# Frikallo/parakeet.cpp

Hardware: AMD Instinct MI355X
Metric: RTFx (audio-sec/wall-sec), mel+encoder+TDT decode, tdt-ctc-110m 10s@b64 (higher is better)
Workload: dtype f32; 1 GPU; tdt-ctc-110m, batch=64x10s clips per GPU, TDT greedy decode (the loops of 4 consecutive steps driven as one lock-step batch), fp32 (BASELINE configs[1]); parallelism=dp1 (utterance shards, no data-path collective), decode_group=4, decode_loop=phases, decode_overlap=1

## Files before the change

include/parakeet_amd.h:

```cpp
#ifndef PARAKEET_AMD_H
#define PARAKEET_AMD_H

#include <stddef.h>
#include <stdint.h>

#ifdef __cplusplus
extern "C" {
#endif

typedef int pk_status;
enum {
    PK_OK = 0,
    PK_ERR_INVALID = -1,
    PK_ERR_IO = -2,
    PK_ERR_WEIGHTS = -3,
    PK_ERR_NO_DEVICE = -4,
    PK_ERR_HIP = -5,
    PK_ERR_DECODE_CAP = -6,
    PK_ERR_UNSUPPORTED = -7
};

typedef struct pk_config {
    int32_t mel_bins;
    int32_t subsampling_channels;
// ... 210 lines not shown
typedef struct pk_sortformer pk_sortformer;
void pk_sortformer_config_preset(pk_sortformer_config *out);
pk_status pk_sortformer_load(const char *safetensors_path, const pk_sortformer_config *cfg, int device, pk_sortformer **out);
void pk_sortformer_free(pk_sortformer *s);
pk_status pk_sortformer_forward(pk_sortformer *s, const float *feats, int B, int Tm, float *probs, int *T_out);
pk_status pk_sortformer_forward_pcm(pk_sortformer *s, const float *pcm, int n_clips, int64_t n_samples, float *probs, int *T_out);
pk_status pk_sortformer_diarize_chunk(pk_sortformer *s, const float *feats, int n_frames, float *probs, int cap_frames, int *T_out);
pk_status pk_sortformer_stream_reset(pk_sortformer *s);
int pk_sortformer_segments(const float *probs, int T, int S, float threshold, int32_t *speaker, float *start, float *end, int cap);

int pk_vocab_size(const pk_model *m);
int pk_detokenize(const pk_model *m, const int32_t *ids, int n, char *out, int cap);
int pk_tokenize(const pk_model *m, const char *text, int32_t *ids, int cap);
pk_status pk_set_boost_tokens(pk_model *m, const int32_t *ids, const int32_t *offsets, int n_phrases, float boost_score);
pk_status pk_set_boost_phrases(pk_model *m, const char *const *phrases, int n_phrases, float boost_score);
int pk_boost_trie_size(const pk_model *m);
int pk_group_timestamps(const pk_model *m, const int32_t *ids, const int32_t *start, const int32_t *end, const float *conf,
                        int n, int sentences, char *words, int cap, float *wstart, float *wend, float *wconf, int wcap);

pk_status pk_diag_math(int fn, const float *in, float *out, int64_t n);
pk_status pk_diag_math_exhaustive(int fn, uint64_t *checked, uint64_t *mismatches, uint64_t *first_bad);
pk_status pk_diag_gemm(int M, int N, int K, const float *A, const float *W, const float *bias, int epi,
                       const float *resid, float alpha, float *out);
pk_status pk_diag_gemm_bf16(int M, int N, int K, const float *A, const float *W, const float *bias, int epi,
                            const float *resid, float alpha, float *out);
pk_status pk_diag_gemm_bf16_a16(int M, int N, int K, const float *A, const float *W, const float *bias, int epi,
                                const float *resid, float alpha, float *out);
pk_status pk_diag_smallm_bf16_tiles(int on);
pk_status pk_diag_ln_gemm_bf16(int M, int N, int K, const float *A, const float *gamma, const float *beta, float eps, const float *W,
                               const float *bias, int epi, const float *resid, float alpha, float *out);
pk_status pk_diag_ln2_gemm_bf16(int M, int N, int K, const float *A, const float *pre_gamma, const float *pre_beta, const float *gamma, const float *beta,
                                float eps, const float *W, const float *bias, float *out, float *pre_out);
pk_status pk_diag_glu_dwconv_bf16(int n_streams, int c, int d, const float *A, const float *gamma, const float *beta, float eps, const float *W,
                                  const float *bias, const float *cache_in, int has_cache, const float *dw_w, const float *dw_bias,
                                  const float *bn_mean, const float *bn_rstd, const float *bn_g, const float *bn_b, int fused, float *out,
                                  float *cache_out);
pk_status pk_diag_ffn_bf16_smallm(int M, int d, int f, const float *x, const float *gamma, const float *beta, float eps, const float *W1, const float *b1,
                                  const float *W2, const float *b2, int act_tiles, float *out);
pk_status pk_diag_layernorm(const float *x, int64_t rows, int d, const float *gamma, const float *beta, float eps, float *y);
pk_status pk_diag_ln_gemm(int M, int N, int K, const float *A, const float *pre_gamma, const float *pre_beta, const float *gamma, const float *beta, float eps,
                          const float *W, const float *bias, int epi, int fold, float *out, float *y1);
pk_status pk_diag_sum64(const float *x, int rows, int n, float *out);
#define PK_DIAG_ATTENTION_GUARD_ROWS 128
pk_status pk_diag_relpos_attention(int kernel, int B, const int32_t *lens, int T, int d, int n_heads, const float *qkv, const float *pos, int pos_T,
                                   const float *bias_u, const float *bias_v, float *ctx, int *variant);
pk_status pk_diag_relpos_local_attention(int B, const int32_t *lens, int T, int d, int n_heads, const float *qkv, const float *pos, int left, int right,
// ... 7 lines not shown
```

parakeet.cpp_amd/capi.py:

```python
import ctypes as C
import os

import numpy as np

from .config import ModelConfig

_HERE = os.path.dirname(os.path.abspath(__file__))
LIB_PATH = os.environ.get("PK_LIB") or os.path.join(_HERE, "libparakeet_amd.so")
_LIB = None

f32p, i32p, i64p = C.POINTER(C.c_float), C.POINTER(C.c_int32), C.POINTER(C.c_int64)


class PkError(RuntimeError):
    def __init__(self, code, msg):
        super().__init__(f"pk_status {code}: {msg}")
        self.code = code


class PkConfig(C.Structure):
    _fields_ = [("mel_bins", C.c_int32), ("subsampling_channels", C.c_int32), ("hidden_size", C.c_int32),
                ("num_layers", C.c_int32), ("num_heads", C.c_int32), ("ffn_intermediate", C.c_int32),
                ("conv_kernel_size", C.c_int32), ("vocab_size", C.c_int32), ("pred_hidden", C.c_int32),
                ("num_lstm_layers", C.c_int32), ("joint_hidden", C.c_int32), ("num_durations", C.c_int32),
# ... 62 lines not shown

def lib():
    global _LIB
    if _LIB is not None:
        return _LIB
    if not os.path.exists(LIB_PATH):
        raise ImportError(f"{LIB_PATH} is missing: run `python -c 'import __graft_entry__ as g; g.build()'` "
                          "(hipcc --offload-arch=gfx950). There is no CPU fallback.")
    L = C.CDLL(LIB_PATH)
    L.pk_version.restype = C.c_char_p
    L.pk_last_error.restype = C.c_size_t
    L.pk_last_error.argtypes = [C.c_char_p, C.c_size_t]
    L.pk_config_preset.argtypes = [C.c_char_p, C.POINTER(PkConfig)]
    L.pk_model_load.argtypes = [C.c_char_p, C.c_char_p, C.POINTER(PkConfig), C.POINTER(C.c_void_p)]
    L.pk_model_to_gpu.argtypes = [C.c_void_p, C.c_int]
    L.pk_model_free.argtypes = [C.c_void_p]
    L.pk_model_config.argtypes = [C.c_void_p, C.POINTER(PkConfig)]
    L.pk_mel.argtypes = [C.c_void_p, f32p, C.c_int, C.c_int64, f32p, f32p]
    L.pk_mel_num_frames.argtypes = [C.c_int64]
    L.pk_encoder_num_frames.argtypes = [C.c_int]
    L.pk_diag_math.argtypes = [C.c_int, f32p, f32p, C.c_int64]
    L.pk_diag_math_exhaustive.argtypes = [C.c_int, C.POINTER(C.c_uint64), C.POINTER(C.c_uint64), C.POINTER(C.c_uint64)]
    L.pk_diag_gemm.argtypes = [C.c_int, C.c_int, C.c_int, f32p, f32p, f32p, C.c_int, f32p, C.c_float, f32p]
    L.pk_diag_gemm_bf16.argtypes = L.pk_diag_gemm.argtypes
    L.pk_diag_gemm_bf16_a16.argtypes = L.pk_diag_gemm.argtypes
    L.pk_diag_layernorm.argtypes = [f32p, C.c_int64, C.c_int, f32p, f32p, C.c_float, f32p]
    L.pk_diag_ln_gemm.argtypes = [C.c_int, C.c_int, C.c_int, f32p, f32p, f32p, f32p, f32p, C.c_float, f32p, f32p, C.c_int, C.c_int, f32p, f32p]
    L.pk_diag_sum64.argtypes = [f32p, C.c_int, C.c_int, f32p]
    L.pk_diag_relpos_attention.argtypes = [C.c_int, C.c_int, i32p, C.c_int, C.c_int, C.c_int, f32p, f32p, C.c_int, f32p, f32p, f32p,
                                           C.POINTER(C.c_int)]
    for name, at in _LATE_SIGNATURES.items():
        if hasattr(L, name):
            getattr(L, name).argtypes = at
    _LIB = L
    return L


_LATE_SIGNATURES = {
    "pk_encode": [C.c_void_p, f32p, C.c_int, C.c_int, C.c_int, C.c_int, f32p],
    "pk_conformer_blocks": [C.c_void_p, f32p, C.c_int, C.c_int, C.c_int, C.c_int, f32p],
    "pk_subsample": [C.c_void_p, f32p, C.c_int, C.c_int, f32p],
    "pk_ctc_decode": [C.c_void_p, f32p, C.c_int, C.c_int, i32p, i32p, i32p, i32p, f32p, f32p],
    "pk_tdt_decode": [C.c_void_p, f32p, C.c_int, C.c_int, C.c_int, i32p, i32p, i32p, i32p, f32p, i32p],
    "pk_model_set_decode_loop": [C.c_void_p, C.c_int],
    "pk_plan_batches": [i64p, C.c_int, i32p, i32p, C.POINTER(C.c_int)],
    "pk_ragged_extents": [i64p, C.c_int, i32p, i32p, i64p],
# ... 156 lines not shown
def read_audio(path, target_rate=16000):
    L = lib()
    L.pk_read_audio.argtypes = [C.c_char_p, C.c_int, C.POINTER(f32p), C.POINTER(C.c_int64), C.POINTER(C.c_int)]
    L.pk_free.argtypes = [C.c_void_p]
    out, n, sr = f32p(), C.c_int64(0), C.c_int(0)
    check(L.pk_read_audio(path.encode(), target_rate, C.byref(out), C.byref(n), C.byref(sr)))
    r = np.ctypeslib.as_array(out, shape=(max(n.value, 1),))[: n.value].copy()
    L.pk_free(out)
    return r, sr.value


def diag_gemm(A, W, bias=None, epi="none", resid=None, alpha=1.0, bf16=False, a16=False):
    A, W = _c(A), _c(W)
    M, K = A.shape
    N = W.shape[0] // 2 if epi == "glu" else W.shape[0]
    b = _c(bias) if bias is not None else None
    r = _c(resid) if resid is not None else None
    out = np.empty((M, N), np.float32)
    fn = (lib().pk_diag_gemm_bf16_a16 if a16 else lib().pk_diag_gemm_bf16) if bf16 else lib().pk_diag_gemm
    check(fn(M, N, K, _f(A), _f(W), _f(b) if b is not None else None, EPI[epi], _f(r) if r is not None else None, alpha, _f(out)))
    return out


def diag_ln_gemm_bf16(A, gamma, beta, W, bias=None, epi="none", resid=None, alpha=1.0, eps=1e-5):
    A, W, gamma, beta = _c(A), _c(W), _c(gamma), _c(beta)
    M, K = A.shape
    N = W.shape[0] // 2 if epi == "glu" else W.shape[0]
    b = _c(bias) if bias is not None else None
    r = _c(resid) if resid is not None else None
    out = np.empty((M, N), np.float32)
    L = lib()
    L.pk_diag_ln_gemm_bf16.argtypes = [C.c_int, C.c_int, C.c_int, f32p, f32p, f32p, C.c_float, f32p, f32p, C.c_int, f32p, C.c_float, f32p]
    check(L.pk_diag_ln_gemm_bf16(M, N, K, _f(A), _f(gamma), _f(beta), eps, _f(W), _f(b) if b is not None else None, EPI[epi],
                                 _f(r) if r is not None else None, alpha, _f(out)))
    return out


def diag_ln2_gemm_bf16(A, pre_gamma, pre_beta, gamma, beta, W, bias, eps=1e-5):
    A, W, pg, pb, g, b, bias = (_c(v) for v in (A, W, pre_gamma, pre_beta, gamma, beta, bias))
    M, K = A.shape
    N = W.shape[0]
    out = np.empty((M, N), np.float32); pre = np.empty((M, K), np.float32)
    L = lib()
    L.pk_diag_ln2_gemm_bf16.argtypes = [C.c_int, C.c_int, C.c_int, f32p, f32p, f32p, f32p, f32p, C.c_float, f32p, f32p, f32p, f32p]
    check(L.pk_diag_ln2_gemm_bf16(M, N, K, _f(A), _f(pg), _f(pb), _f(g), _f(b), eps, _f(W), _f(bias), _f(out), _f(pre)))
    return out, pre
# ... 737 lines not shown
```

parakeet.cpp_amd/csrc/capi.cpp:

```cpp
#include <atomic>
#include <algorithm>
#include <chrono>
#include <cstring>
#include <exception>
#include <functional>
#include <thread>

#include "engine.hpp"
#include "rccl_dyn.hpp"

namespace pk {
const std::string &last_error();
void read_wav(const std::string &path, std::vector<float> &mono, int &sample_rate, int *n_channels = nullptr);
void parse_wav(const uint8_t *bytes, size_t n_bytes, const char *what, std::vector<float> &mono, int &sample_rate, int *n_channels, bool info_only, size_t file_len = 0);
size_t wav_info_frames();
void sinc_resample(const float *input, size_t input_len, int src_rate, int dst_rate, std::vector<float> &output);
}

using namespace pk;

static pk_status guard(const std::function<void()> &fn) {
    try {
        fn();
        return PK_OK;
// ... 1892 lines not shown
        need(K % 32 == 0, "K must be a multiple of 32");
        need(epi >= 0 && epi <= 4, "epi");
        need(epi != EPI_RESID || resid, "resid");
        diag_device();
        const int wrows = epi == EPI_GLU ? 2 * N : N;
        Scratch s;
        s.a.reserve((size_t)M * K * 4);
        s.b.reserve((size_t)wrows * K * 4);
        s.c.reserve((size_t)wrows * 4);
        s.d.reserve((size_t)M * N * 4);
        s.e.reserve((size_t)M * N * 4);
        PK_HIP(hipMemcpy(s.a.p, A, (size_t)M * K * 4, hipMemcpyHostToDevice));
        PK_HIP(hipMemcpy(s.b.p, W, (size_t)wrows * K * 4, hipMemcpyHostToDevice));
        if (bias) PK_HIP(hipMemcpy(s.c.p, bias, (size_t)wrows * 4, hipMemcpyHostToDevice));
        if (resid) PK_HIP(hipMemcpy(s.d.p, resid, (size_t)M * N * 4, hipMemcpyHostToDevice));
        GemmArgs g{s.a.as<float>(), K, s.b.as<float>(), K, bias ? s.c.as<float>() : nullptr, s.e.as<float>(), N,
                   resid ? s.d.as<float>() : nullptr, N, alpha, M, N, K};
        launch_gemm(g, epi, nullptr);
        PK_CHECK_LAUNCH();
        PK_HIP(hipMemcpy(out, s.e.p, (size_t)M * N * 4, hipMemcpyDeviceToHost));
    });
}

static std::atomic<int> g_diag_tiles{1};
pk_status pk_diag_smallm_bf16_tiles(int on) { g_diag_tiles.store(on ? 1 : 0); return PK_OK; }
static const float *diag_operand_tiles(DevBuf &buf, const float *w16, int64_t rows, int K) {
    if (!g_diag_tiles.load() || rows % 16 != 0 || K % 32 != 0) return nullptr;
    buf.reserve((size_t)rows * K * 2);
    launch_tile_copy_bf16(w16, buf.as<float>(), rows, K, K, nullptr);
    return buf.as<float>();
}

pk_status pk_diag_gemm_bf16(int M, int N, int K, const float *A, const float *W, const float *bias, int epi, const float *resid,
                            float alpha, float *out) {
    return guard([&] {
        need(A && W && out && M > 0 && N > 0 && K > 0, "A/W/out/M/N/K");
        need(K % 64 == 0, "K must be a multiple of 64");
        need(epi >= 0 && epi <= 4, "epi");
        need(epi != EPI_RESID || resid, "resid");
        diag_device();
        const int wrows = epi == EPI_GLU ? 2 * N : N;
        std::vector<uint16_t> w16((size_t)wrows * K);
        for (size_t i = 0; i < w16.size(); ++i) {
            uint32_t u;
            memcpy(&u, &W[i], 4);
            u += 0x7fffu + ((u >> 16) & 1u);
// ... 462 lines not shown
```

parakeet.cpp_amd/csrc/kernels/gemm.hip:

```cpp
#include "../pk_devmath.h"
#include "kernels.hpp"
#include <cstdio>
#include <cstdlib>
#include "gemm_pipe.hpp"
#include "gemm_bf16.hpp"
#include "gemm_bf16_glds.hpp"

namespace pk {

typedef float f32x16 __attribute__((ext_vector_type(16)));

static constexpr int BK = 32;
static constexpr int LDP = BK + 1;

template <int BM, int BN, int EPI>
__global__ __launch_bounds__(256) void gemm_nt_kernel(GemmArgs g, int tiles_n, int n_tiles) {
    constexpr int WM = BM / 2, WN = BN / 2;
    constexpr int TM = WM / 32, TN = WN / 32;
    constexpr int A_CH = BM * 8 / 256, W_CH = BN * 8 / 256;
    constexpr int NOUT = (EPI == EPI_GLU) ? BN / 2 : BN;
    static_assert(EPI != EPI_GLU || (TN % 2 == 0), "GLU needs an even number of column tiles per wave");
    extern __shared__ __attribute__((aligned(16))) float smem[];

    int bid = blockIdx.x;
// ... 119 lines not shown
                    float gt = acc[i][j + TN / 2][r];
                    if (g.bias) gt = gt + bias_g;
                    v = v * dsigmoidf(gt);
                }
                if (g.remap_rows) g.out[(int64_t)(row / g.remap_rows) * g.remap_gs + (int64_t)(row % g.remap_rows) * g.remap_rs + (int64_t)col * g.remap_cs] = v;
                else g.out[(int64_t)row * g.ldo + (col < g.sigma_cols ? ((col & ~15) | ((col & 3) << 2) | ((col >> 2) & 3)) : col)] = v;
            }
        }
    }
}

template <int BM, int BN, int EPI>
static void launch_one(const GemmArgs &a, hipStream_t s) {
    constexpr int NOUT = (EPI == EPI_GLU) ? BN / 2 : BN;
    const int tiles_m = (a.M + BM - 1) / BM, tiles_n = (a.N + NOUT - 1) / NOUT;
    const int n_tiles = tiles_m * tiles_n;
    constexpr size_t lds = 2 * (size_t)(BM + BN) * LDP * sizeof(float);
    static DynLdsSlots slots;
    ensure_dyn_lds(slots, reinterpret_cast<const void *>(&gemm_nt_kernel<BM, BN, EPI>), lds);
    hipLaunchKernelGGL((gemm_nt_kernel<BM, BN, EPI>), dim3(n_tiles), dim3(256), lds, s, a, tiles_n, n_tiles);
}

constexpr int kSbSched = 2;
template <int EPI>
static void launch_epi(const GemmArgs &a, hipStream_t s) {
    if (a.K < 64) { launch_one<64, 64, EPI>(a, s); return; }
    const int64_t tiles128 = (int64_t)((a.M + 127) / 128) * ((a.N + 127) / 128);
    if (a.M >= 1024 && a.N >= 256 && a.K >= 1024 && a.K % 64 == 0 && tiles128 <= 256) { launch_gemm_pipe<2, 4, 2, 1, 32, EPI, 1, false, EPI == EPI_NONE ? 0 : kSbSched>(a, s); return; }
    if constexpr (EPI == EPI_NONE || EPI == EPI_RELU || EPI == EPI_SILU) {
        if (a.ln_stats) { launch_gemm_pipe<4, 2, 1, 2, 32, EPI, 1, true, kSbSched>(a, s); return; }
    }
    if (a.M >= 1024 && (a.N >= 1024 || (a.M >= 65536 && a.N >= 256))) launch_gemm_pipe<4, 2, 1, 2, 32, EPI, 1, false, kSbSched>(a, s);
    else if (a.M >= 1024 && a.N >= 256 && a.K >= 1024) launch_gemm_pipe<2, 2, 2, 1, 32, EPI>(a, s);
    else if (a.M >= 1024 && a.N >= 256) launch_gemm_pipe<4, 2, 1, 2, 32, EPI, 1, false, kSbSched>(a, s);
    else launch_gemm_pipe<2, 2, 1, 1, 32, EPI>(a, s);
}

void launch_gemm_smallm(const GemmArgs &a, int epi, hipStream_t s);

bool gemm_ln_stats_applies(const GemmArgs &a, int epi) {
    if (!a.ln_g || !a.ln_b || !a.ln_stats || a.a_bf16 || a.out_bf16 || a.fast_act || a.a_sigma || a.W_sig) return false;
    if (a.M <= kSmallMRows || a.K < 64 || a.K % 32 != 0 || (a.lda & 3) != 0 || (a.ldw & 3) != 0) return false;
    if (epi == EPI_GLU) return true;
    if (epi != EPI_NONE && epi != EPI_RELU && epi != EPI_SILU) return false;
    const int64_t tiles128 = (int64_t)((a.M + 127) / 128) * ((a.N + 127) / 128);
    if (a.K >= 1024 && a.K % 64 == 0 && tiles128 <= 256 && a.N >= 256) return false;
    return a.M >= 1024 && a.N >= 1024;
}

void launch_gemm(const GemmArgs &a, int epi, hipStream_t s) {
    if (a.ln_stats && !gemm_ln_stats_applies(a, epi)) { fprintf(stderr, "parakeet_amd: internal error: GemmArgs::ln_stats on a product the tile kernel does not fold it into\n"); abort(); }
    if (a.M <= kSmallMRows && a.K % 64 == 0) { launch_gemm_smallm(a, epi, s); return; }
    switch (epi) {
    case EPI_NONE: launch_epi<EPI_NONE>(a, s); break;
    case EPI_RELU: launch_epi<EPI_RELU>(a, s); break;
    case EPI_SILU: launch_epi<EPI_SILU>(a, s); break;
    case EPI_RESID: launch_epi<EPI_RESID>(a, s); break;
    case EPI_GLU:
        if (a.K < 64) launch_one<128, 128, EPI_GLU>(a, s);
        else if (a.ln_stats) launch_gemm_pipe<4, 2, 1, 2, 32, EPI_GLU, 1, true, kSbSched>(a, s);
        else launch_gemm_pipe<4, 2, 1, 2, 32, EPI_GLU, 1, false, kSbSched>(a, s);
        break;
    default: break;
    }
}


static bool bf16_glds_rule(int M, int N, int K) {
    return M >= 8192 && N >= 512 && K >= 128 && (int64_t)N * K >= (int64_t)1024 * 1024 && (N & 3) == 0;
}
bool gemm_bf16_blocked_handoff(int M, int N, int K, int epi, bool producer) {
    if (!bf16_glds_rule(M, N, K) || (N % 16) != 0 || (K % 64) != 0) return false;
    if (!producer) return true;
    return epi != EPI_RESID && (int64_t)(M + 31) * N < ((int64_t)1 << 31);
}
[[noreturn]] static void bf16_layout_bug(const char *what) {
    fprintf(stderr, "parakeet_amd: internal error: %s (GemmArgs::out_blocked / a_blocked on a kernel that does not implement it)\n", what);
    abort();
}

template <int EPI, bool A16>
static void launch_bf16_epi(const GemmArgs &a, hipStream_t s) {
    if constexpr (A16) {
        if (a.M >= 8192 && a.N >= 512 && a.K >= 128 && (a.lda % 8) == 0 && (a.ldw % 8) == 0 && a.remap_rows == 0 && (a.ldo & 3) == 0 && (a.N & 3) == 0 &&
            (int64_t)a.N * a.K >= (int64_t)1024 * 1024) {
            constexpr int NOUT = (EPI == EPI_GLU) ? 128 : 256;
            auto est = [&](int R) {
// ... 40 lines not shown
```

parakeet.cpp_amd/csrc/kernels/gemm_pipe.hpp:

```cpp
#ifndef PK_GEMM_PIPE_HPP
#define PK_GEMM_PIPE_HPP
#include <cstdio>
#include <cstdlib>
#include "../pk_devmath.h"
#include "kernels.hpp"

namespace pk {

typedef float gp_f32x16 __attribute__((ext_vector_type(16)));

template <int WGM, int WGN, int TM, int TN, int EPI, int CAP_FLOATS, bool RS_PER_PASS = false, bool EXACT = false>
__device__ __forceinline__ void gp_epilogue(const GemmArgs &g_, gp_f32x16 (&acc)[TM][TN], float *smem, int m0, int n0) {
    struct Flags { int fast_act, out_bf16; };
    const Flags gf{EXACT ? 0 : g_.fast_act, EXACT ? 0 : g_.out_bf16};
    const GemmArgs &g = g_;
    constexpr int NT = 64 * WGM * WGN;
    constexpr int WM = TM * 32, WN = TN * 32, BM = WGM * WM, BN = WGN * WN;
    constexpr int NOUT = (EPI == EPI_GLU) ? BN / 2 : BN;
    const int tid = threadIdx.x, lane = tid & 63, wave = tid >> 6;
    const int wm = wave / WGN, wn = wave % WGN;
    auto epilogue_scalar = [&](int m0, int n0) {
        const int lc = lane & 31, lr = 4 * (lane >> 5);
        constexpr int TNO = (EPI == EPI_GLU) ? TN / 2 : TN;
#pragma unroll
        for (int j = 0; j < TNO; ++j) {
            const int col = n0 + wn * (EPI == EPI_GLU ? WN / 2 : WN) + j * 32 + lc;
            if (col >= g.N) continue;
            const float bias = g.bias ? g.bias[col] : 0.0f;
            float bias_g = 0.0f;
            if constexpr (EPI == EPI_GLU) bias_g = g.bias ? g.bias[g.N + col] : 0.0f;
#pragma unroll
            for (int i = 0; i < TM; ++i) {
#pragma unroll
                for (int r = 0; r < 16; ++r) {
                    const int row = m0 + wm * WM + i * 32 + (r & 3) + 8 * (r >> 2) + lr;
                    if (row >= g.M) continue;
                    float v = acc[i][j][r];
                    if (g.bias) v = v + bias;
                    if constexpr (EPI == EPI_RELU) {
                        v = v > 0.0f ? v : 0.0f;
                    } else if constexpr (EPI == EPI_SILU) {
                        v = gf.fast_act ? fast_siluf(v) : dsiluf(v);
// ... 119 lines not shown
                } else {
                    dsigmoid4(gt);
                }
#pragma unroll
                for (int e = 0; e < 4; ++e) v[e] = v[e] * gt[e];
            }
            if (row < g.M && col_ok) {
                if (gf.out_bf16) {
                    typedef __bf16 bf16x4_ __attribute__((ext_vector_type(4)));
                    const bf16x4_ o = {(__bf16)v[0], (__bf16)v[1], (__bf16)v[2], (__bf16)v[3]};
                    *reinterpret_cast<bf16x4_ *>(reinterpret_cast<__bf16 *>(g.out) + (int64_t)row * g.ldo + col0) = o;
                } else {
                    *reinterpret_cast<float4 *>(g.out + (int64_t)row * g.ldo + col0) = make_float4(v[0], v[1], v[2], v[3]);
                }
            }
        }
        }
    };
    const bool wide = g.remap_rows == 0 && (g.ldo & 3) == 0 && (g.N & 3) == 0 && (EPI != EPI_RESID || (g.ldr & 3) == 0);
    if (wide) epilogue_wide(m0, n0);
    else epilogue_scalar(m0, n0);
}

template <int WGM, int WGN, int TM, int TN, int BK, int EPI, int NBUF = 2, bool LNA = false, int SCHED = 0>
__global__ __launch_bounds__(64 * WGM * WGN) void gemm_pipe_kernel(GemmArgs g, int tiles_n, int n_tiles) {
    static_assert(NBUF == 1 || NBUF == 2, "LDS staging buffers");
    static_assert(SCHED >= 0 && SCHED < 4 && (SCHED == 0 || NBUF == 1), "SCHED: 0..3 k-steps after the second barrier, single-buffered loop only");
    constexpr int NT = 64 * WGM * WGN;
    constexpr int WM = TM * 32, WN = TN * 32, BM = WGM * WM, BN = WGN * WN;
    constexpr int PITCH = BK + 4, BUF = (BM + BN) * PITCH, NSUB = BK / 8, C4R = BK / 4;
    constexpr int A_CH = BM * C4R / NT, W_CH = BN * C4R / NT;
    static_assert(BK == 32 || BK == 64, "BK");
    static_assert((BM * C4R) % NT == 0 && (BN * C4R) % NT == 0, "tile rows must split evenly over the threads");
    constexpr int NOUT = (EPI == EPI_GLU) ? BN / 2 : BN;
    static_assert(EPI != EPI_GLU || (TN % 2 == 0), "GLU needs an even number of column tiles per wave");
    extern __shared__ __attribute__((aligned(16))) float smem[];
    __builtin_amdgcn_s_setprio(3);

    const int tid = threadIdx.x, lane = tid & 63, wave = tid >> 6;
    const int wm = wave / WGN, wn = wave % WGN;
    const int nk = g.K / BK;

    auto chunk_row = [](int c) { const int rr = c / C4R; return (rr & ~7) | ((rr & 1) << 2) | ((rr >> 1) & 3); };
    const float *a_src[A_CH];
    const float *w_src[W_CH];
    int a_dst[A_CH], w_dst[W_CH];
    [[maybe_unused]] float a_mean[LNA ? A_CH : 1], a_rstd[LNA ? A_CH : 1];
    [[maybe_unused]] const float *gam_src = nullptr, *bet_src = nullptr;
    static_assert(!LNA || NT % C4R == 0, "LNA: a thread's chunks share their k offset");
#pragma unroll
    for (int i = 0; i < A_CH; ++i) {
        const int c = tid + NT * i;
        a_dst[i] = chunk_row(c) * PITCH + 2 * (c % C4R);
    }
#pragma unroll
    for (int i = 0; i < W_CH; ++i) {
        const int c = tid + NT * i;
        w_dst[i] = (BM + chunk_row(c)) * PITCH + 2 * (c % C4R);
    }
    auto remap = [&](int b) {
        const int q = n_tiles >> 3, r = n_tiles & 7, xcd = b & 7, idx = b >> 3;
        return (xcd < r ? xcd * (q + 1) : r * (q + 1) + (xcd - r) * q) + idx;
    };
    auto set_tile = [&](int t, int &m0, int &n0) {
        const int bid = remap(t);
        m0 = (bid / tiles_n) * BM;
        n0 = (bid % tiles_n) * NOUT;
#pragma unroll
        for (int i = 0; i < A_CH; ++i) {
            const int c = tid + NT * i;
            int gr = m0 + chunk_row(c);
            gr = gr < g.M ? gr : g.M - 1;
            a_src[i] = g.A + (int64_t)gr * g.lda + (c % C4R) * 4;
            if constexpr (LNA) {
                const float2 st = *reinterpret_cast<const float2 *>(g.ln_stats + 2 * (int64_t)gr);
                a_mean[i] = st.x; a_rstd[i] = st.y;
            }
        }
        if constexpr (LNA) { gam_src = g.ln_g + (tid % C4R) * 4; bet_src = g.ln_b + (tid % C4R) * 4; }
#pragma unroll
        for (int i = 0; i < W_CH; ++i) {
            const int c = tid + NT * i, v = chunk_row(c);
            int wr;
            if constexpr (EPI == EPI_GLU) {
                constexpr int HT = TN / 2;
                const int vw = v / WN, rem = v % WN, tn = rem >> 5, cc = rem & 31;
                int col = n0 + vw * (WN / 2) + (tn % HT) * 32 + cc;
                col = col < g.N ? col : g.N - 1;
                wr = (tn / HT) * g.N + col;
            } else {
                wr = n0 + v;
                wr = wr < g.N ? wr : g.N - 1;
            }
            w_src[i] = g.W + (int64_t)wr * g.ldw + (c % C4R) * 4;
        }
    };

    float4 ra[A_CH], rw[W_CH];
    [[maybe_unused]] float4 rg4, rb4;
    auto gload_chunk = [&](int q, int kt) {
        if (q < A_CH) ra[q] = *reinterpret_cast<const float4 *>(a_src[q] + kt * BK);
        else rw[q - A_CH] = *reinterpret_cast<const float4 *>(w_src[q - A_CH] + kt * BK);
    };
    auto gload = [&](int kt) {
#pragma unroll
        for (int i = 0; i < A_CH; ++i) ra[i] = *reinterpret_cast<const float4 *>(a_src[i] + kt * BK);
#pragma unroll
        for (int i = 0; i < W_CH; ++i) rw[i] = *reinterpret_cast<const float4 *>(w_src[i] + kt * BK);
        if constexpr (LNA) {
            rg4 = *reinterpret_cast<const float4 *>(gam_src + kt * BK);
            rb4 = *reinterpret_cast<const float4 *>(bet_src + kt * BK);
        }
    };
    auto st2 = [&](float *p, float a, float b, float c, float d) {
        if (EPI == EPI_NONE) {
            *reinterpret_cast<float2 *>(p) = make_float2(a, b);
            *reinterpret_cast<float2 *>(p + BK / 2) = make_float2(c, d);
        } else {
            const unsigned addr = (unsigned)(size_t)p;
            asm volatile("ds_write_b32 %0, %1\n\tds_write_b32 %0, %2 offset:4\n\tds_write_b32 %0, %3 offset:%5\n\tds_write_b32 %0, %4 offset:%6"
                         ::"v"(addr), "v"(a), "v"(b), "v"(c), "v"(d), "n"(BK / 2 * 4), "n"(BK / 2 * 4 + 4) : "memory");
        }
    };
    auto lnorm = [&]() {
        if constexpr (LNA) {
            typedef float f2_ __attribute__((ext_vector_type(2)));
            const f2_ g01 = {rg4.x, rg4.y}, g23 = {rg4.z, rg4.w}, b01 = {rb4.x, rb4.y}, b23 = {rb4.z, rb4.w};
#pragma unroll
            for (int i = 0; i < A_CH; ++i) {
                const f2_ m = {a_mean[i], a_mean[i]}, r = {a_rstd[i], a_rstd[i]};
                f2_ lo = {ra[i].x, ra[i].y}, hi = {ra[i].z, ra[i].w};
                lo = __builtin_elementwise_fma((lo - m) * r, g01, b01);
                hi = __builtin_elementwise_fma((hi - m) * r, g23, b23);
                ra[i] = make_float4(lo.x, lo.y, hi.x, hi.y);
            }
        }
// ... 35 lines not shown
        for (int e = 0; e < 4; ++e) {
#pragma unroll
            for (int i = 0; i < TM; ++i) {
                const float a = e == 0 ? fa[slot][i].x : e == 1 ? fa[slot][i].y : e == 2 ? fa[slot][i].z : fa[slot][i].w;
#pragma unroll
                for (int j = 0; j < TN; ++j) {
                    const float b = e == 0 ? fb[slot][j].x : e == 1 ? fb[slot][j].y : e == 2 ? fb[slot][j].z : fb[slot][j].w;
                    acc[i][j] = __builtin_amdgcn_mfma_f32_32x32x2f32(a, b, acc[i][j], 0, 0, 0);
                }
            }
        }
    };
    auto mma_one = [&](int slot, int e, int i, int j) {
        const float a = e == 0 ? fa[slot][i].x : e == 1 ? fa[slot][i].y : e == 2 ? fa[slot][i].z : fa[slot][i].w;
        const float b = e == 0 ? fb[slot][j].x : e == 1 ? fb[slot][j].y : e == 2 ? fb[slot][j].z : fb[slot][j].w;
        acc[i][j] = __builtin_amdgcn_mfma_f32_32x32x2f32(a, b, acc[i][j], 0, 0, 0);
    };
    auto epilogue = [&](int m0, int n0) { gp_epilogue<WGM, WGN, TM, TN, EPI, NBUF * BUF, false, true>(g, acc, smem, m0, n0); };
#define GP_SB() __builtin_amdgcn_sched_barrier(0)
#ifndef GP_LNORM_AT
#define GP_LNORM_AT (NSUB - 2)
#endif

    int m0, n0;
    set_tile(blockIdx.x, m0, n0);
    gload(0);
    lnorm();
    lstore(0);
    lds_store_fence();
    __syncthreads();
    gload(1);
    fragload(0, 0, 0);
    int cur = 0;
    zero_acc();
    if constexpr (NBUF == 1 && SCHED > 0) {
        constexpr int NCH = A_CH + W_CH, E1 = 4 - SCHED, M1 = E1 * TM * TN;
        for (int kt = 0; kt < nk; ++kt) {
            const bool more1 = kt + 1 < nk;
            const int kl = kt + 2 < nk ? kt + 2 : nk - 1;
#pragma unroll
            for (int s = 0; s < NSUB - 1; ++s) {
                fragload(0, s + 1, (s + 1) & 1);
                GP_SB(); mma(s & 1); GP_SB();
                if (LNA && s == GP_LNORM_AT && more1) { lnorm(); GP_SB(); }
            }
            constexpr int SL = (NSUB - 1) & 1;
            __syncthreads();
            GP_SB();
#pragma unroll
            for (int q = 0; q < M1; ++q) {
                const int e = q / (TM * TN), i = (q / TN) % TM, j = q % TN;
                mma_one(SL, e, i, j);
                GP_SB();
#pragma unroll
                for (int c = q * NCH / M1; c < (q + 1) * NCH / M1; ++c) { lstore_chunk(c); GP_SB(); gload_chunk(c, kl); GP_SB(); }
            }
            if constexpr (LNA) {
                rg4 = *reinterpret_cast<const float4 *>(gam_src + kl * BK);
                rb4 = *reinterpret_cast<const float4 *>(bet_src + kl * BK);
                GP_SB();
            }
            lds_store_fence();
            __syncthreads();
            GP_SB();
            fragload(0, 0, 0);
            GP_SB();
#pragma unroll
            for (int e = E1; e < 4; ++e)
#pragma unroll
                for (int i = 0; i < TM; ++i)
#pragma unroll
                    for (int j = 0; j < TN; ++j) mma_one(SL, e, i, j);
            GP_SB();
        }
    } else if constexpr (NBUF == 1) {
        for (int kt = 0; kt < nk; ++kt) {
            const bool more1 = kt + 1 < nk, more2 = kt + 2 < nk;
#pragma unroll
            for (int s = 0; s < NSUB - 1; ++s) {
                fragload(0, s + 1, (s + 1) & 1);
                GP_SB(); mma(s & 1); GP_SB();
                if (LNA && s == GP_LNORM_AT && more1) { lnorm(); GP_SB(); }
            }
            __syncthreads();
            if (more1) lstore(0);
            if (more2) gload(kt + 2);
            GP_SB(); mma((NSUB - 1) & 1); GP_SB();
            lds_store_fence();
            __syncthreads();
            if (more1) fragload(0, 0, 0);
        }
    } else {
        for (int kt = 0; kt < nk; ++kt) {
            const bool more1 = kt + 1 < nk, more2 = kt + 2 < nk;
#pragma unroll
            for (int s = 0; s < NSUB - 1; ++s) {
                fragload(cur, s + 1, (s + 1) & 1);
                if (LNA && s == 0 && more1) lnorm();
                if (s == NSUB - 2 && more1) lstore(cur ^ 1);
                GP_SB(); mma(s & 1); GP_SB();
            }
            lds_store_fence();
            __syncthreads();
            if (more1) fragload(cur ^ 1, 0, 0);
            if (more2) gload(kt + 2);
            GP_SB(); mma((NSUB - 1) & 1); GP_SB();
            cur ^= 1;
        }
    }
    epilogue(m0, n0);
#undef GP_SB
}

template <int WGM, int WGN, int TM, int TN, int BK, int EPI, int NBUF = 2, bool LNA = false, int SCHED = 0>
static void launch_gemm_pipe(const GemmArgs &a, hipStream_t s) {
    constexpr int BM = WGM * TM * 32, BN = WGN * TN * 32;
    constexpr int NOUT = (EPI == EPI_GLU) ? BN / 2 : BN;
    const int tiles_m = (a.M + BM - 1) / BM, tiles_n = (a.N + NOUT - 1) / NOUT;
    const int n_tiles = tiles_m * tiles_n;
    constexpr size_t lds = NBUF * (size_t)(BM + BN) * (BK + 4) * sizeof(float);
    if (a.fast_act || a.out_bf16) { fprintf(stderr, "parakeet_amd: internal error: bf16-mode switches on the fp32 GEMM\n"); abort(); }
    if (LNA != (a.ln_stats != nullptr)) { fprintf(stderr, "parakeet_amd: internal error: GemmArgs::ln_stats on a kernel without the folded LayerNorm (or the reverse)\n"); abort(); }
    auto kern = &gemm_pipe_kernel<WGM, WGN, TM, TN, BK, EPI, NBUF, LNA, SCHED>;
    static DynLdsSlots slots;
    ensure_dyn_lds(slots, reinterpret_cast<const void *>(kern), lds);
    hipLaunchKernelGGL(kern, dim3(n_tiles), dim3(64 * WGM * WGN), lds, s, a, tiles_n, n_tiles);
}

}
#endif
```

parakeet.cpp_amd/csrc/kernels/kernels.hpp:

```cpp
#pragma once
#include <hip/hip_runtime.h>

#include <atomic>
#include <cstdint>

namespace pk {

constexpr int kMaxDevices = 16;
struct DynLdsSlots { std::atomic<size_t> set[kMaxDevices]; };
inline void ensure_dyn_lds(DynLdsSlots &slots, const void *kernel, size_t bytes) {
    int dev = 0;
    (void)hipGetDevice(&dev);
    if (dev < 0 || dev >= kMaxDevices) {
        (void)hipFuncSetAttribute(kernel, hipFuncAttributeMaxDynamicSharedMemorySize, (int)bytes);
        return;
    }
    std::atomic<size_t> &cur = slots.set[dev];
    if (bytes > cur.load(std::memory_order_acquire)) {
        (void)hipFuncSetAttribute(kernel, hipFuncAttributeMaxDynamicSharedMemorySize, (int)bytes);
        cur.store(bytes, std::memory_order_release);
    }
}

struct RagUnit { int b, r0; };
// ... 44 lines not shown
    const float *A; int64_t lda;
    const float *W; int64_t ldw;
    const float *bias;
    float *out; int64_t ldo;
    const float *resid; int64_t ldr; float alpha;
    int M, N, K;
    int remap_rows = 0; int64_t remap_gs = 0, remap_rs = 0, remap_cs = 0;
    int sigma_cols = 0;
    int a_bf16 = 0, out_bf16 = 0;
    int out_blocked = 0, a_blocked = 0;
    int out_t8 = 0, a_t8 = 0;
    int fast_act = 0;
    const float *W_sig = nullptr; int a_sigma = 0;
    const float *W_t16 = nullptr;
    const float *ln_g = nullptr, *ln_b = nullptr; float ln_eps = 0.0f;
    const float *ln_stats = nullptr;
    const float *pre_g = nullptr, *pre_b = nullptr; float *pre_out = nullptr; int64_t pre_ldo = 0;
    const DwTail *dw_tail = nullptr;
};
constexpr int kSmallMRows = 1536;
void launch_sigma_copy(const float *src, float *dst, int64_t rows, int K, int64_t ld, hipStream_t s);
void launch_tile_copy_bf16(const float *src16, float *dst16, int64_t rows, int K, int64_t ld, hipStream_t s);
void launch_gemm(const GemmArgs &a, int epi, hipStream_t s);
bool gemm_ln_stats_applies(const GemmArgs &a, int epi);
bool gemm_bf16_blocked_handoff(int M, int N, int K, int epi, bool producer);
bool gemm_smallm_ln_applies(const GemmArgs &a, int epi);
bool gemm_smallm_pre_applies(const GemmArgs &a, int epi);
bool gemm_smallm_dw_applies(const GemmArgs &a, int epi, int c, int kc);
void launch_gemm_bf16(const GemmArgs &a, int epi, hipStream_t s);
constexpr int kSmallMRowsBf16 = 128;
bool gemm_smallm_bf16_applies(const GemmArgs &a, int epi);
bool gemm_smallm_bf16_dw_applies(const GemmArgs &a, int epi, int c, int kc);
bool gemm_smallm_bf16_ln_applies(const GemmArgs &a, int epi);
bool gemm_smallm_bf16_pre_applies(const GemmArgs &a, int epi);
void launch_gemm_smallm_bf16(const GemmArgs &a, int epi, hipStream_t s);
double gemm_flops(const GemmArgs &a, int epi);

int sub_conv1_dw1_strip_rows(int64_t total_h2_rows);
void launch_sub_conv1_dw1(const float *feats, int B, int Tm, int F, int C, const float *w1, const float *b1, const float *wd,
                          const float *bd, float *out, hipStream_t s, const SubRag &rag = SubRag());
void launch_sub_dw(const float *in, int B, int H, int W, int C, const float *wd, const float *bd, float *out, hipStream_t s, const SubRag &rag = SubRag());

size_t relpos_attention_lds_bytes(int T, int hd);
int relpos_attention_max_frames(int hd);
size_t relpos_attention_scratch_bytes(int B, int T, int n_heads, int hd);
void launch_relpos_attention(const float *qkv, int B, int T, int d, int n_heads, const float *pos, const float *bias_u,
// ... 138 lines not shown
```

Before: 36270 x real-time.

## Make the LayerNorm-folded fp32 GEMM persistent and overlap next-tile loads with the epilogue

```diff
diff --git a/include/parakeet_amd.h b/include/parakeet_amd.h
--- a/include/parakeet_amd.h
+++ b/include/parakeet_amd.h
@@ -256,6 +256,7 @@
 pk_status pk_diag_math_exhaustive(int fn, uint64_t *checked, uint64_t *mismatches, uint64_t *first_bad);
 pk_status pk_diag_gemm(int M, int N, int K, const float *A, const float *W, const float *bias, int epi,
                        const float *resid, float alpha, float *out);
+pk_status pk_diag_gemm_plan(int M, int N, int K, int epi, int ln_fold, int *plan);
 pk_status pk_diag_gemm_bf16(int M, int N, int K, const float *A, const float *W, const float *bias, int epi,
                             const float *resid, float alpha, float *out);
 pk_status pk_diag_gemm_bf16_a16(int M, int N, int K, const float *A, const float *W, const float *bias, int epi,
diff --git a/parakeet.cpp_amd/capi.py b/parakeet.cpp_amd/capi.py
--- a/parakeet.cpp_amd/capi.py
+++ b/parakeet.cpp_amd/capi.py
@@ -108,6 +108,7 @@
     L.pk_diag_math.argtypes = [C.c_int, f32p, f32p, C.c_int64]
     L.pk_diag_math_exhaustive.argtypes = [C.c_int, C.POINTER(C.c_uint64), C.POINTER(C.c_uint64), C.POINTER(C.c_uint64)]
     L.pk_diag_gemm.argtypes = [C.c_int, C.c_int, C.c_int, f32p, f32p, f32p, C.c_int, f32p, C.c_float, f32p]
+    L.pk_diag_gemm_plan.argtypes = [C.c_int, C.c_int, C.c_int, C.c_int, C.c_int, C.POINTER(C.c_int)]
     L.pk_diag_gemm_bf16.argtypes = L.pk_diag_gemm.argtypes
     L.pk_diag_gemm_bf16_a16.argtypes = L.pk_diag_gemm.argtypes
     L.pk_diag_layernorm.argtypes = [f32p, C.c_int64, C.c_int, f32p, f32p, C.c_float, f32p]
@@ -310,6 +311,12 @@
     return out
 
 
+def diag_gemm_plan(M, N, K, epi="none", ln_fold=False):
+    p = (C.c_int * 7)()
+    check(lib().pk_diag_gemm_plan(M, N, K, EPI[epi], int(bool(ln_fold)), p))
+    return dict(zip(("tile_kernel", "bm", "bn", "n_tiles", "grid", "persist", "resident"), (int(v) for v in p)))
+
+
 def diag_ln_gemm_bf16(A, gamma, beta, W, bias=None, epi="none", resid=None, alpha=1.0, eps=1e-5):
     A, W, gamma, beta = _c(A), _c(W), _c(gamma), _c(beta)
     M, K = A.shape
diff --git a/parakeet.cpp_amd/csrc/capi.cpp b/parakeet.cpp_amd/csrc/capi.cpp
--- a/parakeet.cpp_amd/csrc/capi.cpp
+++ b/parakeet.cpp_amd/csrc/capi.cpp
@@ -1938,6 +1938,20 @@
     });
 }
 
+pk_status pk_diag_gemm_plan(int M, int N, int K, int epi, int ln_fold, int *plan) {
+    return guard([&] {
+        need(plan && M > 0 && N > 0 && K > 0 && K % 32 == 0, "plan/M/N/K");
+        need(epi >= 0 && epi <= 4, "epi");
+        diag_device();
+        static float dummy[4];
+        GemmArgs g{dummy, K, dummy, K, dummy, dummy, N, epi == EPI_RESID ? dummy : nullptr, N, 1.0f, M, N, K};
+        if (ln_fold) { g.ln_g = dummy; g.ln_b = dummy; g.ln_stats = dummy; }
+        GemmPlan p;
+        const bool tile = gemm_plan(g, epi, &p);
+        plan[0] = tile ? 1 : 0; plan[1] = p.bm; plan[2] = p.bn; plan[3] = p.n_tiles; plan[4] = p.grid; plan[5] = p.persist; plan[6] = p.resident;
+    });
+}
+
 static std::atomic<int> g_diag_tiles{1};
 pk_status pk_diag_smallm_bf16_tiles(int on) { g_diag_tiles.store(on ? 1 : 0); return PK_OK; }
 static const float *diag_operand_tiles(DevBuf &buf, const float *w16, int64_t rows, int K) {
diff --git a/parakeet.cpp_amd/csrc/kernels/gemm.hip b/parakeet.cpp_amd/csrc/kernels/gemm.hip
--- a/parakeet.cpp_amd/csrc/kernels/gemm.hip
+++ b/parakeet.cpp_amd/csrc/kernels/gemm.hip
@@ -165,17 +165,27 @@
 }
 
 constexpr int kSbSched = 2;
+template <int EPI, bool LNA>
+constexpr bool kSbPersist = EPI == EPI_NONE && LNA;
+template <int EPI, bool LNA>
+static void launch_wide_sb(const GemmArgs &a, hipStream_t s) {
+    if constexpr (kSbPersist<EPI, LNA>) {
+        const int64_t tiles = (int64_t)((a.M + 127) / 128) * ((a.N + (EPI == EPI_GLU ? 63 : 127)) / (EPI == EPI_GLU ? 64 : 128));
+        if (tiles > gp_resident_slots()) { launch_gemm_pipe<4, 2, 1, 2, 32, EPI, 1, LNA, kSbSched, true>(a, s); return; }
+    }
+    launch_gemm_pipe<4, 2, 1, 2, 32, EPI, 1, LNA, kSbSched>(a, s);
+}
 template <int EPI>
 static void launch_epi(const GemmArgs &a, hipStream_t s) {
     if (a.K < 64) { launch_one<64, 64, EPI>(a, s); return; }
     const int64_t tiles128 = (int64_t)((a.M + 127) / 128) * ((a.N + 127) / 128);
     if (a.M >= 1024 && a.N >= 256 && a.K >= 1024 && a.K % 64 == 0 && tiles128 <= 256) { launch_gemm_pipe<2, 4, 2, 1, 32, EPI, 1, false, EPI == EPI_NONE ? 0 : kSbSched>(a, s); return; }
     if constexpr (EPI == EPI_NONE || EPI == EPI_RELU || EPI == EPI_SILU) {
-        if (a.ln_stats) { launch_gemm_pipe<4, 2, 1, 2, 32, EPI, 1, true, kSbSched>(a, s); return; }
-    }
-    if (a.M >= 1024 && (a.N >= 1024 || (a.M >= 65536 && a.N >= 256))) launch_gemm_pipe<4, 2, 1, 2, 32, EPI, 1, false, kSbSched>(a, s);
+        if (a.ln_stats) { launch_wide_sb<EPI, true>(a, s); return; }
+    }
+    if (a.M >= 1024 && (a.N >= 1024 || (a.M >= 65536 && a.N >= 256))) launch_wide_sb<EPI, false>(a, s);
     else if (a.M >= 1024 && a.N >= 256 && a.K >= 1024) launch_gemm_pipe<2, 2, 2, 1, 32, EPI>(a, s);
-    else if (a.M >= 1024 && a.N >= 256) launch_gemm_pipe<4, 2, 1, 2, 32, EPI, 1, false, kSbSched>(a, s);
+    else if (a.M >= 1024 && a.N >= 256) launch_wide_sb<EPI, false>(a, s);
     else launch_gemm_pipe<2, 2, 1, 1, 32, EPI>(a, s);
 }
 
@@ -201,11 +211,23 @@
     case EPI_RESID: launch_epi<EPI_RESID>(a, s); break;
     case EPI_GLU:
         if (a.K < 64) launch_one<128, 128, EPI_GLU>(a, s);
-        else if (a.ln_stats) launch_gemm_pipe<4, 2, 1, 2, 32, EPI_GLU, 1, true, kSbSched>(a, s);
-        else launch_gemm_pipe<4, 2, 1, 2, 32, EPI_GLU, 1, false, kSbSched>(a, s);
+        else if (a.ln_stats) launch_wide_sb<EPI_GLU, true>(a, s);
+        else launch_wide_sb<EPI_GLU, false>(a, s);
         break;
     default: break;
     }
+}
+
+bool gemm_plan(const GemmArgs &a, int epi, GemmPlan *plan) {
+    GemmPipePlan p{0, 0, 0, 0, 0};
+    *plan = GemmPlan{0, 0, 0, 0, 0, gp_resident_slots()};
+    if ((a.M <= kSmallMRows && a.K % 64 == 0) || a.K < 64 || epi < EPI_NONE || epi > EPI_GLU) return false;
+    if (a.ln_stats && !gemm_ln_stats_applies(a, epi)) return false;
+    gp_dry_run = &p;
+    launch_gemm(a, epi, nullptr);
+    gp_dry_run = nullptr;
+    *plan = GemmPlan{p.bm, p.bn, p.n_tiles, p.grid, p.persist, gp_resident_slots()};
+    return p.n_tiles > 0;
 }
 
 
diff --git a/parakeet.cpp_amd/csrc/kernels/gemm_pipe.hpp b/parakeet.cpp_amd/csrc/kernels/gemm_pipe.hpp
--- a/parakeet.cpp_amd/csrc/kernels/gemm_pipe.hpp
+++ b/parakeet.cpp_amd/csrc/kernels/gemm_pipe.hpp
@@ -2,6 +2,7 @@
 #define PK_GEMM_PIPE_HPP
 #include <cstdio>
 #include <cstdlib>
+#include <type_traits>
 #include "../pk_devmath.h"
 #include "kernels.hpp"
 
@@ -9,15 +10,28 @@
 
 typedef float gp_f32x16 __attribute__((ext_vector_type(16)));
 
+#ifdef GP_TRACE
+constexpr int GP_TRACE_TILES = 10, GP_TRACE_SLOTS = 32;
+__device__ long long *gp_trace;
+#define GP_STAMP(slot) do { if (gp_trace && threadIdx.x == 0 && (slot) < GP_TRACE_SLOTS) gp_trace[(long long)blockIdx.x * GP_TRACE_SLOTS + (slot)] = wall_clock64(); } while (0)
+#define GP_STAMP_TILE(i, ph) do { if ((i) < GP_TRACE_TILES) GP_STAMP(2 + 3 * (i) + (ph)); } while (0)
+#define GP_STAMP_HWID() do { if (gp_trace && threadIdx.x == 0) { const unsigned hw_ = __builtin_amdgcn_s_getreg((31 << 11) | 4), xcc_ = __builtin_amdgcn_s_getreg((3 << 11) | 20); \
+        gp_trace[(long long)blockIdx.x * GP_TRACE_SLOTS] = (long long)hw_ | ((long long)xcc_ << 32); } } while (0)
+#else
+#define GP_STAMP(slot) do { } while (0)
+#define GP_STAMP_TILE(i, ph) do { } while (0)
+#define GP_STAMP_HWID() do { } while (0)
+#endif
+
 template <int WGM, int WGN, int TM, int TN, int EPI, int CAP_FLOATS, bool RS_PER_PASS = false, bool EXACT = false>
-__device__ __forceinline__ void gp_epilogue(const GemmArgs &g_, gp_f32x16 (&acc)[TM][TN], float *smem, int m0, int n0) {
+__device__ __forceinline__ void gp_epilogue(const GemmArgs &g_, gp_f32x16 (&acc)[TM][TN], float *smem, int m0, int n0, int tid_ = threadIdx.x) {
     struct Flags { int fast_act, out_bf16; };
     const Flags gf{EXACT ? 0 : g_.fast_act, EXACT ? 0 : g_.out_bf16};
     const GemmArgs &g = g_;
     constexpr int NT = 64 * WGM * WGN;
     constexpr int WM = TM * 32, WN = TN * 32, BM = WGM * WM, BN = WGN * WN;
     constexpr int NOUT = (EPI == EPI_GLU) ? BN / 2 : BN;
-    const int tid = threadIdx.x, lane = tid & 63, wave = tid >> 6;
+    const int tid = tid_, lane = tid & 63, wave = tid >> 6;
     const int wm = wave / WGN, wn = wave % WGN;
     auto epilogue_scalar = [&](int m0, int n0) {
         const int lc = lane & 31, lr = 4 * (lane >> 5);
@@ -183,9 +197,10 @@
     else epilogue_scalar(m0, n0);
 }
 
-template <int WGM, int WGN, int TM, int TN, int BK, int EPI, int NBUF = 2, bool LNA = false, int SCHED = 0>
-__global__ __launch_bounds__(64 * WGM * WGN) void gemm_pipe_kernel(GemmArgs g, int tiles_n, int n_tiles) {
+template <int WGM, int WGN, int TM, int TN, int BK, int EPI, int NBUF = 2, bool LNA = false, int SCHED = 0, bool PERSIST = false>
+__global__ __launch_bounds__(64 * WGM * WGN, PERSIST ? 4 : 0) void gemm_pipe_kernel(GemmArgs g, int tiles_n, int n_tiles) {
     static_assert(NBUF == 1 || NBUF == 2, "LDS staging buffers");
+    static_assert(!PERSIST || (NBUF == 1 && SCHED > 0), "PERSIST: the hand-placed single-buffered loop only");
     static_assert(SCHED >= 0 && SCHED < 4 && (SCHED == 0 || NBUF == 1), "SCHED: 0..3 k-steps after the second barrier, single-buffered loop only");
     constexpr int NT = 64 * WGM * WGN;
     constexpr int WM = TM * 32, WN = TN * 32, BM = WGM * WM, BN = WGN * WN;
@@ -223,7 +238,8 @@
         const int q = n_tiles >> 3, r = n_tiles & 7, xcd = b & 7, idx = b >> 3;
         return (xcd < r ? xcd * (q + 1) : r * (q + 1) + (xcd - r) * q) + idx;
     };
-    auto set_tile = [&](int t, int &m0, int &n0) {
+    auto set_tile = [&](int t, int &m0, int &n0, auto with_ln) {
+        constexpr bool WITH_LN = decltype(with_ln)::value;
         const int bid = remap(t);
         m0 = (bid / tiles_n) * BM;
         n0 = (bid % tiles_n) * NOUT;
@@ -233,7 +249,7 @@
             int gr = m0 + chunk_row(c);
             gr = gr < g.M ? gr : g.M - 1;
             a_src[i] = g.A + (int64_t)gr * g.lda + (c % C4R) * 4;
-            if constexpr (LNA) {
+            if constexpr (LNA && WITH_LN) {
                 const float2 st = *reinterpret_cast<const float2 *>(g.ln_stats + 2 * (int64_t)gr);
                 a_mean[i] = st.x; a_rstd[i] = st.y;
             }
@@ -257,22 +273,37 @@
         }
     };
 
+    [[maybe_unused]] auto set_tile_ln = [&](int m0) {
+        if constexpr (LNA) {
+#pragma unroll
+            for (int i = 0; i < A_CH; ++i) {
+                int gr = m0 + chunk_row(tid + NT * i);
+                gr = gr < g.M ? gr : g.M - 1;
+                const float2 st = *reinterpret_cast<const float2 *>(g.ln_stats + 2 * (int64_t)gr);
+                a_mean[i] = st.x; a_rstd[i] = st.y;
+            }
+        }
+    };
+
     float4 ra[A_CH], rw[W_CH];
     [[maybe_unused]] float4 rg4, rb4;
     auto gload_chunk = [&](int q, int kt) {
         if (q < A_CH) ra[q] = *reinterpret_cast<const float4 *>(a_src[q] + kt * BK);
         else rw[q - A_CH] = *reinterpret_cast<const float4 *>(w_src[q - A_CH] + kt * BK);
     };
-    auto gload = [&](int kt) {
-#pragma unroll
-        for (int i = 0; i < A_CH; ++i) ra[i] = *reinterpret_cast<const float4 *>(a_src[i] + kt * BK);
-#pragma unroll
-        for (int i = 0; i < W_CH; ++i) rw[i] = *reinterpret_cast<const float4 *>(w_src[i] + kt * BK);
+    [[maybe_unused]] auto gload_ln = [&](int kt) {
         if constexpr (LNA) {
             rg4 = *reinterpret_cast<const float4 *>(gam_src + kt * BK);
             rb4 = *reinterpret_cast<const float4 *>(bet_src + kt * BK);
         }
     };
+    auto gload_aw = [&](int kt) {
+#pragma unroll
+        for (int i = 0; i < A_CH; ++i) ra[i] = *reinterpret_cast<const float4 *>(a_src[i] + kt * BK);
+#pragma unroll
+        for (int i = 0; i < W_CH; ++i) rw[i] = *reinterpret_cast<const float4 *>(w_src[i] + kt * BK);
+    };
+    auto gload = [&](int kt) { gload_aw(kt); gload_ln(kt); };
     auto st2 = [&](float *p, float a, float b, float c, float d) {
         if (EPI == EPI_NONE) {
             *reinterpret_cast<float2 *>(p) = make_float2(a, b);
@@ -354,18 +385,24 @@
 #define GP_LNORM_AT (NSUB - 2)
 #endif
 
+    auto first_ktile = [&]() {
+        lnorm();
+        lstore(0);
+        lds_store_fence();
+        __syncthreads();
+        gload(1);
+        fragload(0, 0, 0);
+        zero_acc();
+    };
     int m0, n0;
-    set_tile(blockIdx.x, m0, n0);
+    GP_STAMP_HWID();
+    GP_STAMP(1);
+    set_tile(blockIdx.x, m0, n0, std::true_type{});
     gload(0);
-    lnorm();
-    lstore(0);
-    lds_store_fence();
-    __syncthreads();
-    gload(1);
-    fragload(0, 0, 0);
-    int cur = 0;
-    zero_acc();
-    if constexpr (NBUF == 1 && SCHED > 0) {
+    first_ktile();
+    GP_STAMP_TILE(0, 0);
+    [[maybe_unused]] int cur = 0;
+    [[maybe_unused]] auto kloop_sched = [&]() {
         constexpr int NCH = A_CH + W_CH, E1 = 4 - SCHED, M1 = E1 * TM * TN;
         for (int kt = 0; kt < nk; ++kt) {
             const bool more1 = kt + 1 < nk;
@@ -405,6 +442,30 @@
                     for (int j = 0; j < TN; ++j) mma_one(SL, e, i, j);
             GP_SB();
         }
+    };
+    if constexpr (PERSIST) {
+        int t = blockIdx.x;
+        for ([[maybe_unused]] int it = 0;; ++it) {
+            kloop_sched();
+            GP_STAMP_TILE(it, 1);
+            const int tn = t + (int)gridDim.x, em0 = m0, en0 = n0;
+            const bool more = tn < n_tiles;
+            if (more) { set_tile(tn, m0, n0, std::false_type{}); gload_aw(0); }
+            int tid_e = tid;
+            asm volatile("" : "+v"(tid_e));
+            gp_epilogue<WGM, WGN, TM, TN, EPI, NBUF * BUF, false, true>(g, acc, smem, em0, en0, tid_e);
+            GP_STAMP_TILE(it, 2);
+            if (!more) break;
+            t = tn;
+            set_tile_ln(m0);
+            gload_ln(0);
+            __syncthreads();
+            first_ktile();
+            GP_STAMP_TILE(it + 1, 0);
+        }
+        return;
+    } else if constexpr (NBUF == 1 && SCHED > 0) {
+        kloop_sched();
     } else if constexpr (NBUF == 1) {
         for (int kt = 0; kt < nk; ++kt) {
             const bool more1 = kt + 1 < nk, more2 = kt + 2 < nk;
@@ -440,23 +501,46 @@
             cur ^= 1;
         }
     }
+    GP_STAMP_TILE(0, 1);
     epilogue(m0, n0);
+    GP_STAMP_TILE(0, 2);
 #undef GP_SB
 }
 
-template <int WGM, int WGN, int TM, int TN, int BK, int EPI, int NBUF = 2, bool LNA = false, int SCHED = 0>
+struct GemmPipePlan { int bm, bn, n_tiles, grid, persist; };
+inline thread_local GemmPipePlan *gp_dry_run = nullptr;
+
+inline int gp_cu_count() {
+    static std::atomic<int> cus[kMaxDevices];
+    int dev = 0;
+    (void)hipGetDevice(&dev);
+    const bool slot = dev >= 0 && dev < kMaxDevices;
+    int n = slot ? cus[dev].load(std::memory_order_acquire) : 0;
+    if (n <= 0) {
+        if (hipDeviceGetAttribute(&n, hipDeviceAttributeMultiprocessorCount, dev) != hipSuccess || n <= 0) { fprintf(stderr, "parakeet_amd: cannot read the device's compute unit count\n"); abort(); }
+        if (slot) cus[dev].store(n, std::memory_order_release);
+    }
+    return n;
+}
+inline int gp_resident_slots() { return 2 * gp_cu_count(); }
+
+template <int WGM, int WGN, int TM, int TN, int BK, int EPI, int NBUF = 2, bool LNA = false, int SCHED = 0, bool PERSIST = false>
 static void launch_gemm_pipe(const GemmArgs &a, hipStream_t s) {
     constexpr int BM = WGM * TM * 32, BN = WGN * TN * 32;
     constexpr int NOUT = (EPI == EPI_GLU) ? BN / 2 : BN;
+    static_assert(!PERSIST || 64 * WGM * WGN == 512, "PERSIST: the grid is sized for two 512-thread workgroups per CU");
     const int tiles_m = (a.M + BM - 1) / BM, tiles_n = (a.N + NOUT - 1) / NOUT;
     const int n_tiles = tiles_m * tiles_n;
     constexpr size_t lds = NBUF * (size_t)(BM + BN) * (BK + 4) * sizeof(float);
     if (a.fast_act || a.out_bf16) { fprintf(stderr, "parakeet_amd: internal error: bf16-mode switches on the fp32 GEMM\n"); abort(); }
     if (LNA != (a.ln_stats != nullptr)) { fprintf(stderr, "parakeet_amd: internal error: GemmArgs::ln_stats on a kernel without the folded LayerNorm (or the reverse)\n"); abort(); }
-    auto kern = &gemm_pipe_kernel<WGM, WGN, TM, TN, BK, EPI, NBUF, LNA, SCHED>;
+    int grid = n_tiles;
+    if constexpr (PERSIST) { const int res = gp_resident_slots(); grid = n_tiles < res ? n_tiles : res; }
+    if (gp_dry_run) { *gp_dry_run = GemmPipePlan{BM, BN, n_tiles, grid, PERSIST ? 1 : 0}; return; }
+    auto kern = &gemm_pipe_kernel<WGM, WGN, TM, TN, BK, EPI, NBUF, LNA, SCHED, PERSIST>;
     static DynLdsSlots slots;
     ensure_dyn_lds(slots, reinterpret_cast<const void *>(kern), lds);
-    hipLaunchKernelGGL(kern, dim3(n_tiles), dim3(64 * WGM * WGN), lds, s, a, tiles_n, n_tiles);
+    hipLaunchKernelGGL(kern, dim3(grid), dim3(64 * WGM * WGN), lds, s, a, tiles_n, n_tiles);
 }
 
 }
diff --git a/parakeet.cpp_amd/csrc/kernels/kernels.hpp b/parakeet.cpp_amd/csrc/kernels/kernels.hpp
--- a/parakeet.cpp_amd/csrc/kernels/kernels.hpp
+++ b/parakeet.cpp_amd/csrc/kernels/kernels.hpp
@@ -90,6 +90,8 @@
 void launch_sigma_copy(const float *src, float *dst, int64_t rows, int K, int64_t ld, hipStream_t s);
 void launch_tile_copy_bf16(const float *src16, float *dst16, int64_t rows, int K, int64_t ld, hipStream_t s);
 void launch_gemm(const GemmArgs &a, int epi, hipStream_t s);
+struct GemmPlan { int bm, bn, n_tiles, grid, persist, resident; };
+bool gemm_plan(const GemmArgs &a, int epi, GemmPlan *plan);
 bool gemm_ln_stats_applies(const GemmArgs &a, int epi);
 bool gemm_bf16_blocked_handoff(int M, int N, int K, int epi, bool producer);
 bool gemm_smallm_ln_applies(const GemmArgs &a, int epi);
```

New measurement: 36320 x real-time, median of 6. No clear change (+0.1%).
